# chenchen235/SemStereo

Measured on AMD Instinct MI355X. Metric: stereo pairs/sec, hot segment (gwc+concat volumes, 3-D hourglass stack, soft-argmax), 1024x1024 maxdisp=128, higher is better.
Workload: dtype f32; 1 GPU; BASELINE.json configs[1]: 1024x1024, maxdisp=128, batch=1/GPU x 1 GPU(s); features [B,128,H/4,W/4]+[B,256,H/8,W/8] -> disparity; input_sets_rotated=3, execution=steps round-robin on 6 HIP streams (PairPipeline); bit-identical to one stream, conv_engine=f16x3, hip_graph=False

## Files before the change

### include/semstereo_hip.h

```cpp
#ifndef SEMSTEREO_HIP_H
#define SEMSTEREO_HIP_H

#ifdef __cplusplus
extern "C" {
#endif

typedef void* ss_stream_t;

enum ss_status {
    SS_OK = 0,
    SS_ERR_INVALID = -1,
    SS_ERR_UNSUPPORTED = -2,
    SS_ERR_LAUNCH = -3
};

int ss_abi_version(void);
int ss_reload_tuning(void);
int ss_set_fill_hint(int pairs_in_flight);
int ss_get_fill_hint(void);
const char* ss_status_string(int status);
const char* ss_last_hip_error(void);


int ss_groupwise_correlation_fwd(const float* fea1, const float* fea2, float* out,
                                 int B, int C, int H, int W, int groups, int normalize,
                                 ss_stream_t stream);

int ss_gwc_volume_fwd(const float* ref, const float* tgt, float* out,
                      int B, int C, int H, int W, int dmin, int ndisp, int groups, int normalize,
                      ss_stream_t stream);
int ss_gwc_patch_gate_fwd(const float* ref, const float* tgt, const float* patch_w, const float* gate_logits, float* out,
                          int B, int C, int H, int W, int dmin, int ndisp, int groups, int normalize, ss_stream_t stream);
int ss_gwc_volume_bwd(const float* grad_out, const float* ref, const float* tgt,
                      float* grad_ref, float* grad_tgt,
                      int B, int C, int H, int W, int dmin, int ndisp, int groups,
                      ss_stream_t stream);

int ss_concat_volume_fwd(const float* ref, const float* tgt, float* out,
                         int B, int C, int H, int W, int dmin, int ndisp, int mask_left, ss_stream_t stream);
int ss_concat_volume_bwd(const float* grad_out, float* grad_ref, float* grad_tgt,
                         int B, int C, int H, int W, int dmin, int ndisp, int mask_left, ss_stream_t stream);

int ss_warp_sampled_fwd(const float* x, const float* y, const float* disp,
                        float* y_warped, float* x_warped,
                        int B, int C, int H, int W, int nd, ss_stream_t stream);
int ss_warp_sampled_bwd(const float* grad_y_warped, const float* grad_x_warped, const float* y, const float* disp,
                        float* grad_x, float* grad_y, float* grad_disp, int B, int C, int H, int W, int nd,
                        ss_stream_t stream);
int ss_concat_sampled_fwd(const float* left, const float* right, const float* disp, const float* att,
                          float* out, int B, int C, int H, int W, int nd, ss_stream_t stream);
int ss_concat_sampled_bwd(const float* grad_out, const float* left, const float* right, const float* disp, const float* att,
                          float* grad_left, float* grad_right, float* grad_att, int B, int C, int H, int W, int nd, int margin,
                          ss_stream_t stream);
int ss_concat_sampled_presplit_fwd(const float* right, const float* disp, const float* att, void* xs, int* xexp,
                                   int B, int C, int H, int W, int nd, ss_stream_t stream);
int ss_stem_left_fwd(const float* q, const float* att, float* out, int B, int Cout, int nd, int H, int W,
                     ss_stream_t stream);
int ss_stem_left_fused_fwd(const float* left, const void* wsplit, const float* att, float* out, int B, int C,
                           int Cout, int nd, int H, int W, int nterms, ss_stream_t stream);
int ss_warp_correlation_fwd(const float* x, const float* y, const float* disp, float* out,
                            int B, int C, int H, int W, int nd, ss_stream_t stream);

int ss_disparity_regression_fwd(const float* prob, float* out, int B, int dmin, int ndisp, int H, int W,
                                ss_stream_t stream);
int ss_disparity_regression_bwd(const float* grad_out, float* grad_prob, int B, int dmin, int ndisp, int H, int W,
                                ss_stream_t stream);
int ss_disparity_variance_fwd(const float* prob, const float* disparity, float* out,
                              int B, int dmin, int ndisp, int H, int W, ss_stream_t stream);
int ss_softmax_regression_fwd(const float* logits, float* prob, float* disp, float* var,
                              int B, int dmin, int ndisp, int H, int W, ss_stream_t stream);
int ss_upsample_softmax_regression_fwd(const float* coarse, float* up, float* disp, float* var,
                                       int B, int dmin, int ndisp, int H, int W, ss_stream_t stream);

int ss_sample_strength_fwd(const float* left, const float* right, const float* pred0, const float* var,
                           const float* gamma, const float* beta, float* strength,
                           int B, int C, int H, int W, ss_stream_t stream);
int ss_topk_candidates_fwd(const float* logits, const float* strength, float* samples, float* att_topk,
                           float* pred_att, int B, int dmin, int ndisp, int H, int W, int k, ss_stream_t stream);

int ss_regression_topk_fwd(const float* cost, const float* samples, float* out,
                           int B, int nd, int H, int W, int k, ss_stream_t stream);
int ss_regression_topk_bwd(const float* grad_out, const float* cost, const float* samples, float* grad_cost,
                           float* grad_samples, int B, int nd, int H, int W, int k, ss_stream_t stream);

int ss_ssr_upsample_fwd(const float* depth_low, const float* weights, const float* pred_label,
                        const float* params, float* out, int B, int h, int w, int num_classes,
                        ss_stream_t stream);
int ss_ssr_param_count(void);
int ss_ssr_upsample_train_fwd(const float* depth_low, const float* weights, const float* pred_label, const float* params,
                              float* out, float* saved, float* rm0, float* rv0, long long* nbt0, float* rma, float* rva,
                              long long* nbta, float* rm1, float* rv1, long long* nbt1, float* rm2, float* rv2, long long* nbt2,
                              float eps0, float epsa, float eps1, float eps2, double mom0, double moma, double mom1, double mom2,
                              int batch_stats, int B, int h, int w, int num_classes, double* workspace, long long workspace_bytes,
                              ss_stream_t stream);
int ss_ssr_upsample_train_bwd(const float* depth_low, const float* weights, const float* pred_label, const float* params,
                              const float* saved, const float* grad_out, float* grad_depth_low, float* grad_weights,
                              float* grad_pred_label, float* grad_params, int batch_stats, int B, int h, int w, int num_classes,
                              double* workspace, long long workspace_bytes, ss_stream_t stream);

int ss_channel_gate_fwd(const float* att_logits, const float* cv, float* out,
                        int B, int C, int D, int H, int W, ss_stream_t stream);

int ss_channel_att_logits_fwd(const float* im, const void* w1_split, const float* scale1, const float* shift1,
                              const void* w2_split, const float* bias2, float* out,
                              int B, int Cin, int Cmid, int Cout, int H, int W, int sigmoid, ss_stream_t stream);

int ss_conv3d_fwd(const float* in, const float* wpack, const float* scale, const float* shift,
                  const float* residual, const float* gate, float* out,
                  int B, int Cin, int D, int H, int W, int Cout, int k, int stride, int relu,
                  ss_stream_t stream);
int ss_conv3d_bf16s_fwd(const float* in, const void* wsplit, const float* scale, const float* shift,
                        const float* residual, const float* gate, float* out,
// ... 167 lines not shown
```

### semstereo_amd/_lib.py

```python
import ctypes
import os

import torch

_HERE = os.path.dirname(os.path.abspath(__file__))
LIB_PATH = os.path.join(_HERE, "csrc", "libsemstereo_hip.so")
ABI_VERSION = 20

_P = ctypes.c_void_p
_I = ctypes.c_int

_SIGNATURES = {
    "ss_groupwise_correlation_fwd": [_P, _P, _P, _I, _I, _I, _I, _I, _I, _P],
    "ss_gwc_volume_fwd": [_P, _P, _P, _I, _I, _I, _I, _I, _I, _I, _I, _P],
    "ss_gwc_patch_gate_fwd": [_P, _P, _P, _P, _P, _I, _I, _I, _I, _I, _I, _I, _I, _P],
    "ss_gwc_volume_bwd": [_P, _P, _P, _P, _P, _I, _I, _I, _I, _I, _I, _I, _P],
    "ss_concat_volume_fwd": [_P, _P, _P, _I, _I, _I, _I, _I, _I, _I, _P],
    "ss_concat_volume_bwd": [_P, _P, _P, _I, _I, _I, _I, _I, _I, _I, _P],
    "ss_warp_sampled_fwd": [_P, _P, _P, _P, _P, _I, _I, _I, _I, _I, _P],
    "ss_warp_sampled_bwd": [_P, _P, _P, _P, _P, _P, _P, _I, _I, _I, _I, _I, _P],
    "ss_concat_sampled_fwd": [_P, _P, _P, _P, _P, _I, _I, _I, _I, _I, _P],
    "ss_concat_sampled_bwd": [_P, _P, _P, _P, _P, _P, _P, _P, _I, _I, _I, _I, _I, _I, _P],
    "ss_concat_sampled_presplit_fwd": [_P, _P, _P, _P, _P, _I, _I, _I, _I, _I, _P],
    "ss_conv3d_presplit_fwd": [_P, _P, _P, _P, _P, _P, _P, _P, _I, _I, _I, _I, _I, _I, _I, _P],
    "ss_stem_left_fwd": [_P, _P, _P, _I, _I, _I, _I, _I, _P],
    "ss_stem_left_fused_fwd": [_P, _P, _P, _P, _I, _I, _I, _I, _I, _I, _I, _P],
    "ss_warp_correlation_fwd": [_P, _P, _P, _P, _I, _I, _I, _I, _I, _P],
    "ss_disparity_regression_fwd": [_P, _P, _I, _I, _I, _I, _I, _P],
    "ss_disparity_regression_bwd": [_P, _P, _I, _I, _I, _I, _I, _P],
    "ss_disparity_variance_fwd": [_P, _P, _P, _I, _I, _I, _I, _I, _P],
    "ss_softmax_regression_fwd": [_P, _P, _P, _P, _I, _I, _I, _I, _I, _P],
    "ss_upsample_softmax_regression_fwd": [_P, _P, _P, _P, _I, _I, _I, _I, _I, _P],
    "ss_regression_topk_fwd": [_P, _P, _P, _I, _I, _I, _I, _I, _P],
    "ss_regression_topk_bwd": [_P, _P, _P, _P, _P, _I, _I, _I, _I, _I, _P],
    "ss_sample_strength_fwd": [_P, _P, _P, _P, _P, _P, _P, _I, _I, _I, _I, _P],
    "ss_topk_candidates_fwd": [_P, _P, _P, _P, _P, _I, _I, _I, _I, _I, _I, _P],
    "ss_channel_gate_fwd": [_P, _P, _P, _I, _I, _I, _I, _I, _P],
    "ss_channel_att_logits_fwd": [_P, _P, _P, _P, _P, _P, _P, _I, _I, _I, _I, _I, _I, _I, _P],
    "ss_ssr_upsample_fwd": [_P, _P, _P, _P, _P, _I, _I, _I, _I, _P],
    "ss_ssr_upsample_train_fwd": [_P, _P, _P, _P, _P, _P] + [_P] * 12 + [ctypes.c_float] * 4 + [ctypes.c_double] * 4
                                 + [_I, _I, _I, _I, _I, _P, ctypes.c_longlong, _P],
    "ss_ssr_upsample_train_bwd": [_P] * 10 + [_I, _I, _I, _I, _I, _P, ctypes.c_longlong, _P],
    "ss_conv3d_fwd": [_P, _P, _P, _P, _P, _P, _P, _I, _I, _I, _I, _I, _I, _I, _I, _I, _P],
    "ss_conv3d_bf16s_fwd": [_P, _P, _P, _P, _P, _P, _P, _I, _I, _I, _I, _I, _I, _I, _I, _I, _P],
    "ss_conv3d_bf16s_partial_fwd": [_P, _P, _P, _P, _P, _P, _P, _I, _I, _I, _I, _I, _I, _I, _I, _P],
    "ss_conv3d_gather_fwd": [_P, _P, _P, _P, _P, _P, _P, _P, _P, _I, _I, _I, _I, _I, _I, _I, _I, _P],
    "ss_pack_conv3d_weights_bf16s": [_P, _P, _I, _I, _P],
    "ss_pack_conv3d_weights_f16s": [_P, _P, _I, _I, _P],
    "ss_conv2d_bf16s_fwd": [_P, _P, _P, _P, _P, _P, _I, _I, _I, _I, _I, _I, _I, _P],
    "ss_conv2d_bf16s_pair_fwd": [_P, _P, _P, _P, _P, _P, _I, _I, _I, _I, _I, _I, _I, _P],
    "ss_pack_conv2d_weights_bf16s": [_P, _P, _I, _I, _P],
    "ss_conv2d_bf16s_cat_fwd": [_P, _P, _P, _P, _P, _P, _P, _P, _I, _I, _I, _I, _I, _I, _I, _I, _P],
    "ss_deconv2d_bf16s_fwd": [_P, _P, _P, _P, _P, _I, _I, _I, _I, _I, _I, _I, _P],
    "ss_deconv2d_bf16s_pair_fwd": [_P, _P, _P, _P, _P, _P, _I, _I, _I, _I, _I, _I, _I, _P],
    "ss_pack_deconv2d_weights_f16s": [_P, _P, _I, _I, _P],
    "ss_pack_conv2d_weights_f16s": [_P, _P, _I, _I, _P],
    "ss_conv2d_k1_f16s_fwd": [_P, _P, _P, _P, _P, _I, _I, ctypes.c_longlong, _I, _I, _P],
    "ss_conv2d_k1_f16s_pair_fwd": [_P, _P, _P, _P, _P, _P, _I, _I, ctypes.c_longlong, _I, _I, _P],
    "ss_pack_conv2d_k1_weights_f16s": [_P, _P, _I, _I, _P],
    "ss_seghead_logits_fwd": [_P, _P, _P, _P, _P, _P, _P, _I, _I, _I, _I, _I, _P],
    "ss_pack_seghead_weights_f16s": [_P, _P, _I, _P],
    "ss_bilinear_up2_fwd": [_P, _P, _I, _I, _I, _I, _P],
    "ss_conv3d_head_bf16s_fwd": [_P, _P, _P, _P, _P, _I, _I, _I, _I, _I, _I, _I, _P],
    "ss_conv3d_head_bf16s_cl_fwd": [_P, _P, _P, _P, _P, _I, _I, _I, _I, _I, _I, _I, _P],
    "ss_conv3d_bf16s_cl_fwd": [_P, _P, _P, _P, _P, _I, _I, _I, _I, _I, _I, _I, _I, _P],
    "ss_pack_classifier_head_weights": [_P, _P, _P],
    "ss_conv3d_classifier_fused_fwd": [_P, _P, _P, _P, _P, _P, _P, _I, _I, _I, _I, _I, _I, _P],
    "ss_regression_topk_patched_fwd": [_P, _P, _P, _I, _I, _I, _I, _I, _P],
    "ss_pack_conv3d_head_weights_bf16s": [_P, _P, _I, _P],
    "ss_pack_conv3d_head_weights_f16s": [_P, _P, _I, _P],
    "ss_conv3d_pointwise_bf16s_fwd": [_P, _P, _P, _P, _P, _I, _I, _I, ctypes.c_longlong, _I, _I, _P],
    "ss_pack_pointwise_weights_bf16s": [_P, _P, _I, _I, _P],
    "ss_deconv3d_fwd": [_P, _P, _P, _P, _P, _P, _P, _P, _P, _I, _I, _I, _I, _I, _I, _I, _I, _P],
    "ss_pack_deconv3d_weights_f16s": [_P, _P, _I, _I, _P],
    "ss_deconv3d_bf16s_fwd": [_P, _P, _P, _P, _P, _P, _I, _I, _I, _I, _I, _I, _I, _I, _I, _P],
    "ss_pack_deconv3d_weights_bf16s": [_P, _P, _I, _I, _I, _P],
    "ss_pack_conv3d_weights": [_P, _P, _I, _I, _I, _I, _P],
    "ss_conv3d_wgrad_fwd": [_P, _P, _P, _I, _I, _I, _I, _I, _I, _I, _P],
    "ss_conv3d_wgrad_bf16s_fwd": [_P, _P, _P, _P, _I, _I, _I, _I, _I, _I, _I, _P],
# ... 107 lines not shown
```

### semstereo_amd/csrc/stem_left.hip

```cpp
#include <algorithm>

#include "common.h"
#include "split_bf16.h"

namespace {

constexpr int TH = 8, TW = 32, COG = 4;

template <int ND>
__global__ __launch_bounds__(256) void stem_left_kernel(const float* __restrict__ q, const float* __restrict__ att,
                                                         float* __restrict__ out, int Cout, int H, int W) {
    __shared__ float atile[ND][TH + 2][TW + 2];
    const int tid = threadIdx.x, tx = tid & 31, ty = tid >> 5;
    const int w0 = blockIdx.x * TW, h0 = blockIdx.y * TH;
    const int ngroups = Cout / COG;
    const int b = blockIdx.z / ngroups, co0 = (blockIdx.z % ngroups) * COG;
    const size_t plane = (size_t)H * W;
    const float* ab = att + (size_t)b * ND * plane;
    for (int e = tid; e < ND * (TH + 2) * (TW + 2); e += 256) {
        const int x = e % (TW + 2);
        int r = e / (TW + 2);
        const int y = r % (TH + 2), j = r / (TH + 2);
        const int gh = h0 + y - 1, gw = w0 + x - 1;
        atile[j][y][x] = ((unsigned)gh < (unsigned)H && (unsigned)gw < (unsigned)W) ? ab[(size_t)j * plane + (size_t)gh * W + gw] : 0.f;
    }
    __syncthreads();
    const int h = h0 + ty, w = w0 + tx;
    if (h >= H || w >= W) return;
    float acc[COG][ND];
#pragma unroll
    for (int c = 0; c < COG; ++c)
#pragma unroll
        for (int j = 0; j < ND; ++j) acc[c][j] = 0.f;
    const float* qb = q + ((size_t)b * 27 * Cout + co0) * plane;
    float qv[2][3][COG];
    auto load_q = [&](float (&dst)[3][COG], int s) {
        const int kh = s / 3, kw = s % 3;
        const int y = min(max(h + kh - 1, 0), H - 1), x = min(max(w + kw - 1, 0), W - 1);
        const float* p = qb + (size_t)y * W + x;
#pragma unroll
        for (int kd = 0; kd < 3; ++kd)
#pragma unroll
            for (int c = 0; c < COG; ++c) dst[kd][c] = p[((size_t)((kd * 3 + kh) * 3 + kw) * Cout + c) * plane];
    };
    load_q(qv[0], 0);
#pragma unroll
    for (int s = 0; s < 9; ++s) {
        if (s + 1 < 9) load_q(qv[(s + 1) & 1], s + 1);
        const int kh = s / 3, kw = s % 3;
        float a[ND + 2];
        a[0] = 0.f;
        a[ND + 1] = 0.f;
#pragma unroll
        for (int j = 0; j < ND; ++j) a[1 + j] = atile[j][ty + kh][tx + kw];
#pragma unroll
        for (int kd = 0; kd < 3; ++kd)
// ... 164 lines not shown
                const int qrow = ((kd * 3 + kh) * 3 + kw) * 2;
                const f32x2_t v = {qtile[qrow][hp], qtile[qrow + 1][hp]};
#pragma unroll
                for (int j = 0; j < NJ; ++j) o[j] = __builtin_elementwise_fma(f32x2_t{av[j + kd], av[j + kd]}, v, o[j]);
            }
        }
        if (inside) {
            float* ob = out + (((size_t)b * Cout + 2 * g) * ND + j0) * plane + (size_t)h * W + w;
#pragma unroll
            for (int j = 0; j < NJ; ++j) {
                ob[(size_t)j * plane] = o[j][0];
                ob[((size_t)ND + j) * plane] = o[j][1];
            }
        }
    }
}

template <int ND>
int launch_fused(const float* left, const void* wsplit, const float* att, float* out, int B, int Cout, int H, int W,
                 int nterms, hipStream_t st) {
    const size_t lds = ((size_t)(ND + 2) * HH * HW + 64 * QCOLS) * sizeof(float);
    dim3 grid(ss::ceil_div(W, FTW), ss::ceil_div(H, FTH), B);
    if (nterms == 6) {
        auto kern = stem_left_fused<ND, 6>;
        if (lds > 64 * 1024) {
            if (ss::ensure_dynamic_lds(reinterpret_cast<const void*>(kern), (int)lds) != SS_OK) return SS_ERR_LAUNCH;
        }
        hipLaunchKernelGGL(kern, grid, dim3(256), lds, st, left, reinterpret_cast<const uint4*>(wsplit), att, out, Cout, H, W);
    } else {
        auto kern = stem_left_fused<ND, 3>;
        if (lds > 64 * 1024) {
            if (ss::ensure_dynamic_lds(reinterpret_cast<const void*>(kern), (int)lds) != SS_OK) return SS_ERR_LAUNCH;
        }
        hipLaunchKernelGGL(kern, grid, dim3(256), lds, st, left, reinterpret_cast<const uint4*>(wsplit), att, out, Cout, H, W);
    }
    return ss::check_launch();
}

}

extern "C" int ss_stem_left_fused_fwd(const float* left, const void* wsplit, const float* att, float* out, int B, int C,
                                      int Cout, int nd, int H, int W, int nterms, ss_stream_t stream) {
    SS_REQUIRE(left && wsplit && att && out);
    SS_REQUIRE(B > 0 && C > 0 && Cout > 0 && nd > 0 && H > 0 && W > 0 && (nterms == 3 || nterms == 6));
    SS_REQUIRE((reinterpret_cast<uintptr_t>(wsplit) & 15) == 0);
    if (C != 32 || Cout % 2 != 0 || B > 65535) return SS_ERR_UNSUPPORTED;
    if ((long long)C * H * W * 4 >= 0x7fffffffLL || (long long)nd * H * W * 4 >= 0x7fffffffLL) return SS_ERR_UNSUPPORTED;
    hipStream_t st = ss::as_stream(stream);
    if (nd == 24) return launch_fused<24>(left, wsplit, att, out, B, Cout, H, W, nterms, st);
    if (nd == 32) return launch_fused<32>(left, wsplit, att, out, B, Cout, H, W, nterms, st);
    if (nd == 6) return launch_fused<6>(left, wsplit, att, out, B, Cout, H, W, nterms, st);
    return SS_ERR_UNSUPPORTED;
}
```

### semstereo_amd/engine.py

```python
import os
import weakref

import torch
import torch.nn as nn

from . import _lib, ops
from ._lib import call, ptr

PATH_COUNTS = {"hip": 0, "torch": 0}


def _inference(module, *tensors):
    if module.training:
        return False
    if torch.is_grad_enabled():
        if any(t is not None and t.requires_grad for t in tensors):
            return False
        if any(p.requires_grad for p in module.parameters()):
            return False
        if module.__dict__.get("_is_replica", False):
            for m in module.modules():
                if any(p is not None and p.requires_grad for p in getattr(m, "_former_parameters", {}).values()):
                    return False
    return True
# ... 562 lines not shown
    w = w.detach().float().reshape(w.shape[0], w.shape[1]).contiguous()
    _lib.require_device(w)
    Cout, Cin = w.shape
    assert Cin % 16 == 0
    out = torch.empty(((Cout + 31) // 32) * (Cin // 16) * 3 * 2 * 32 * 8, dtype=torch.int16, device=w.device)
    with torch.cuda.device(w.device):
        call("ss_pack_pointwise_weights_bf16s", ptr(w), ptr(out), Cout, Cin)
    return out


def conv3d_pointwise_bf16s_hip(x, wsplit, Cout, scale, shift, relu, nterms):
    x = x if x.is_contiguous() else x.contiguous()
    dev = _lib.require_device(x, scale, shift)
    B, Cin = x.shape[0], x.shape[1]
    out = torch.empty((B, Cout) + tuple(x.shape[2:]), dtype=x.dtype, device=x.device)
    with torch.cuda.device(dev):
        call("ss_conv3d_pointwise_bf16s_fwd", ptr(x), ptr(wsplit), ptr(scale), ptr(shift), ptr(out), B, Cin, Cout,
             x[0, 0].numel(), int(relu), int(nterms))
    return out


def _conv_geometry(conv):
    k, s, p = conv.kernel_size, conv.stride, conv.padding
    assert k[0] == k[1] == k[2] and s[0] == s[1] == s[2] and p[0] == p[1] == p[2] == k[0] // 2
    assert conv.bias is None and conv.groups == 1 and conv.dilation == (1, 1, 1)
    return k[0], s[0]


def run_convbn(owner, key, conv, bn, x, relu, residual=None, gate=None):
    k, s = _conv_geometry(conv)
    if CONV_ENGINE != "f32" and k == 3 and s in (1, 2) and conv.out_channels > 1:
        nterms = _tiled_nterms()
        ws, scale, shift = _packed_affine(owner, key + ("/f16s" if nterms == 19 else "/bf16s"), conv, bn,
                                          lambda w: pack_conv_weight_bf16s(w, nterms))
        return conv3d_bf16s_hip(x, ws, conv.out_channels, scale, shift, relu, nterms, residual, gate, stride=s)
    if (CONV_ENGINE != "f32" and k == 3 and s == 1 and conv.out_channels == 1 and conv.in_channels in (16, 32, 64)
            and residual is None and gate is None):
        nterms = _head_nterms()
        ws, scale, shift = _packed_affine(owner, key + "/head_%d" % nterms, conv, bn, lambda w: pack_head_weight_bf16s(w, nterms))
        return conv3d_head_bf16s_hip(x, ws, scale, shift, relu, nterms)
    wp, scale, shift = _packed_affine(owner, key, conv, bn, pack_conv_weight)
    return conv3d_hip(x, wp, scale, shift, k, s, relu, residual, gate)


TRAIN_HIP = os.environ.get("SS_TRAIN_HIP", "1") != "0"
SSR_TRAIN_HIP = os.environ.get("SS_SSR_TRAIN_HIP", "1") != "0"
LOSS_HIP = os.environ.get("SS_LOSS_HIP", "1") != "0"
METRICS_HIP = os.environ.get("SS_METRICS_HIP", "1") != "0"
CLASSIFIER_CL = os.environ.get("SS_CLASSIFIER_CL", "1") != "0"
CLASSIFIER_FUSED = os.environ.get("SS_CLASSIFIER_FUSED", "1") != "0"


STEM_LEFT_FUSED = os.environ.get("SS_STEM_LEFT_FUSED", "1") != "0"


def _stem_halves_params(stem, C):
    conv, bn = stem.conv, stem.bn if stem.use_bn else None
    Cout = conv.out_channels
    assert conv.in_channels == 2 * C and _conv_geometry(conv) == (3, 1)
    srcs = [conv.weight] + ([bn.weight, bn.bias, bn.running_mean, bn.running_var] if bn is not None else [])

    def build():
        sc, sh = fold_bn(bn) if bn is not None else (None, None)
        w = conv.weight.detach().float()
        wl = w[:, :C].reshape(Cout, C, 27)
        wq = wl.permute(2, 0, 1).reshape(27 * Cout, C)
        wf = torch.zeros(Cout // 2, 64, C, dtype=w.dtype, device=w.device)
        wf[:, :54] = wl.reshape(Cout // 2, 2, C, 27).permute(0, 3, 1, 2).reshape(Cout // 2, 54, C)
        return (pack_pointwise_weight_bf16s(wq), pack_pointwise_weight_bf16s(wf.reshape(Cout // 2 * 64, C)),
                pack_conv_weight_bf16s(w[:, C:].contiguous(), _tiled_nterms()), sc, sh)
    return _cache(stem).get("bc/halves/" + CONV_ENGINE, srcs, build)


def stem_broadcast_half(stem, left, att):
    assert stem.is_3d and not stem.deconv and CONV_ENGINE != "f32" and _inference(stem, left, att)
    C, Cout = left.shape[1], stem.conv.out_channels
    nterms = _aux_nterms()
    wq, wf, _, _, _ = _stem_halves_params(stem, C)
    PATH_COUNTS["hip"] += 1
    if C == 32 and Cout % 2 == 0 and STEM_LEFT_FUSED:
        return ops.stem_left_fused(left, wf, att, Cout, nterms)
    q = conv3d_pointwise_bf16s_hip(left, wq, 27 * Cout, None, None, False, nterms)
    return ops.stem_left(q, att)


def stem_volume_half(stem, right_vol, partial, gate=None):
    assert stem.is_3d and not stem.deconv and CONV_ENGINE != "f32" and _inference(stem, right_vol, partial, gate)
    nterms = _tiled_nterms()
    _, _, wr, scale, shift = _stem_halves_params(stem, right_vol.shape[1])
    g = None if gate is None else gate.contiguous()
    return conv3d_bf16s_hip(right_vol, wr, stem.conv.out_channels, scale, shift, bool(stem.relu), nterms, None, g, partial=partial)


STEM_PRESPLIT = os.environ.get("SS_STEM_PRESPLIT", "0") != "0"


def stem_presplit_applies(stem, right):
    return (STEM_PRESPLIT and CONV_ENGINE == "f16x3" and right.shape[1] % 8 == 0 and stem.conv.in_channels == 2 * right.shape[1]
            and _conv_geometry(stem.conv) == (3, 1))


def stem_volume_half_presplit(stem, xs, xexp, partial, gate=None):
    assert stem.is_3d and not stem.deconv and CONV_ENGINE == "f16x3" and _inference(stem, partial, gate)
    B, nchunks, _, D, H, W, _ = xs.shape
    _, _, wr, scale, shift = _stem_halves_params(stem, nchunks * 8)
    Cout = stem.conv.out_channels
    g = None if gate is None else gate.contiguous()
    dev = _lib.require_device(partial, scale, shift, g)
    out = torch.empty((B, Cout, D, H, W), dtype=torch.float32, device=xs.device)
    if partial is not None:
        assert partial.shape == out.shape and partial.is_contiguous()
    with torch.cuda.device(dev if dev is not None else xs.device):
        call("ss_conv3d_presplit_fwd", ptr(xs), ptr(xexp), ptr(wr), ptr(partial), ptr(scale), ptr(shift), ptr(g), ptr(out),
             B, nchunks * 8, D, H, W, Cout, int(bool(stem.relu)))
    return out


STEM_GATHER = os.environ.get("SS_STEM_GATHER", "1") != "0"
STEM_INPLACE = os.environ.get("SS_STEM_INPLACE", "1") != "0"


def stem_gather_applies(stem, right, samples):
    return (STEM_GATHER and CONV_ENGINE == "f16x3" and right.shape[1] % 8 == 0 and right.shape[1] >= 16
            and stem.conv.in_channels == 2 * right.shape[1] and _conv_geometry(stem.conv) == (3, 1)
            and right.dtype == torch.float32 and samples.dtype == torch.float32
            and right.shape[-1] > 1 and right.shape[-2] > 1)


def stem_gather_half(stem, right, samples, att, partial, gate=None, consume_partial=False):
    assert stem.is_3d and not stem.deconv and CONV_ENGINE == "f16x3" and _inference(stem, right, partial, gate)
    right, samples = right.contiguous(), samples.contiguous()
    att = att.reshape(att.shape[0], att.shape[-3], att.shape[-2], att.shape[-1]).contiguous()
    B, C, H, W = right.shape
    nd = samples.shape[1]
    assert samples.shape == (B, nd, H, W) and att.shape == samples.shape
    _, _, wr, scale, shift = _stem_halves_params(stem, C)
    Cout = stem.conv.out_channels
    g = None if gate is None else gate.contiguous()
    dev = _lib.require_device(right, samples, att, partial, scale, shift, g)
    inplace = consume_partial and STEM_INPLACE and partial is not None and partial.is_contiguous() and tuple(partial.shape) == (B, Cout, nd, H, W) and not partial.requires_grad
    out = partial if inplace else torch.empty((B, Cout, nd, H, W), dtype=torch.float32, device=right.device)
    if partial is not None:
        assert partial.shape == out.shape and partial.is_contiguous()
    if g is not None:
        assert g.shape == (B, Cout, H, W)
    PATH_COUNTS["hip"] += 1
    with torch.cuda.device(dev):
        call("ss_conv3d_gather_fwd", ptr(right), ptr(samples), ptr(att), ptr(wr), ptr(partial), ptr(scale), ptr(shift), ptr(g),
             ptr(out), B, C, nd, H, W, Cout, int(bool(stem.relu)), _tiled_nterms())
    return out


def stem_of_broadcast_and_volume(stem, left, att, right_vol, gate=None):
    return stem_volume_half(stem, right_vol, stem_broadcast_half(stem, left, att), gate)

ATTENTION_FORM = os.environ.get("SS_ATTENTION", "split")

SWITCHES = ("CONV_ENGINE", "DECONV_F16", "DECONV_MIN_WORKGROUPS", "DECONV_BF16S", "CLASSIFIER_CL", "CLASSIFIER_FUSED", "CLASSIFIER_FOLD", "TRAIN_HIP", "SSR_TRAIN_HIP", "LOSS_HIP", "METRICS_HIP", "ATTENTION_FORM",
            "STEM_LEFT_FUSED", "STEM_PRESPLIT", "STEM_GATHER", "STEM_INPLACE", "HEAD_F16", "CONV2D_HIP", "DECODER_HIP", "HEADS_HIP")
```

### semstereo_amd/ops.py

```python
import torch
import torch.nn.functional as F

from . import _lib
from . import deferred as dfr
from ._lib import call, ptr


def _c(t):
    return t if t.is_contiguous() else t.contiguous()


def _needs_grad(*ts):
    return torch.is_grad_enabled() and any(t is not None and t.requires_grad for t in ts)



def signed_range(maxdisp):
    return -int(maxdisp), 2 * int(maxdisp)


def unsigned_range(maxdisp):
    return 0, int(maxdisp)


# ... 377 lines not shown
def concat_volume_sampled(left, right, disparity_samples, att=None):
    right, disp = _c(right), _c(disparity_samples)
    left = None if left is None else _c(left)
    if att is not None:
        att = _c(att.reshape(att.shape[0], att.shape[-3], att.shape[-2], att.shape[-1]))
    dev = _lib.require_device(left, right, disp, att)
    B, C, H, W = right.shape
    nd = disp.shape[1]
    out = torch.empty((B, (2 if left is not None else 1) * C, nd, H, W), dtype=right.dtype, device=right.device)
    with torch.cuda.device(dev):
        call("ss_concat_sampled_fwd", ptr(left), ptr(right), ptr(disp), ptr(att), ptr(out), B, C, H, W, nd)
    return out


def concat_volume_sampled_presplit(right, disparity_samples, att=None):
    right, disp = _c(right), _c(disparity_samples)
    if att is not None:
        att = _c(att.reshape(att.shape[0], att.shape[-3], att.shape[-2], att.shape[-1]))
    dev = _lib.require_device(right, disp, att)
    B, C, H, W = right.shape
    nd = disp.shape[1]
    assert C % 8 == 0
    xs = torch.empty((B, C // 8, 2, nd, H, W, 8), dtype=torch.int16, device=right.device)
    xexp = torch.empty(3 * B, dtype=torch.int32, device=right.device)
    with torch.cuda.device(dev):
        call("ss_concat_sampled_presplit_fwd", ptr(right), ptr(disp), ptr(att), ptr(xs), ptr(xexp), B, C, H, W, nd)
    return xs, xexp


def stem_left(q, att):
    q = _c(q)
    att = _c(att.reshape(att.shape[0], att.shape[-3], att.shape[-2], att.shape[-1]))
    dev = _lib.require_device(q, att)
    B, nd, H, W = att.shape
    assert q.shape[0] == B and q.shape[1] % 27 == 0 and tuple(q.shape[2:]) == (H, W)
    Cout = q.shape[1] // 27
    out = torch.empty((B, Cout, nd, H, W), dtype=q.dtype, device=q.device)
    with torch.cuda.device(dev):
        call("ss_stem_left_fwd", ptr(q), ptr(att), ptr(out), B, Cout, nd, H, W)
    return out


def stem_left_fused(left, wsplit, att, Cout, nterms=6):
    left = _c(left)
    att = _c(att.reshape(att.shape[0], att.shape[-3], att.shape[-2], att.shape[-1]))
    dev = _lib.require_device(left, att)
    B, nd, H, W = att.shape
    out = torch.empty((B, Cout, nd, H, W), dtype=left.dtype, device=left.device)
    with torch.cuda.device(dev):
        call("ss_stem_left_fused_fwd", ptr(left), ptr(wsplit), ptr(att), ptr(out), B, left.shape[1], Cout, nd, H, W, int(nterms))
    return out


def warp_correlation(x, y, disparity_samples):
    x, y, disp = _c(x), _c(y), _c(disparity_samples)
    dev = _lib.require_device(x, y, disp)
    B, C, H, W = x.shape
    nd = disp.shape[1]
    out = torch.empty((B, nd, H, W), dtype=x.dtype, device=x.device)
    with torch.cuda.device(dev):
        call("ss_warp_correlation_fwd", ptr(x), ptr(y), ptr(disp), ptr(out), B, C, H, W, nd)
    return out


def sample_strength(left, right, pred0, var, gamma, beta):
    left, right, pred0, var = _c(left), _c(right), _c(pred0), _c(var)
    gamma, beta = _c(gamma.detach().reshape(1)), _c(beta.detach().reshape(1))
    dev = _lib.require_device(left, right, pred0, var, gamma, beta)
    B, C, H, W = left.shape
    assert pred0.shape == (B, H, W) and var.shape == (B, 1, H, W)
    out = torch.empty((B, 5, H, W), dtype=left.dtype, device=left.device)
    with torch.cuda.device(dev):
        call("ss_sample_strength_fwd", ptr(left), ptr(right), ptr(pred0), ptr(var), ptr(gamma), ptr(beta), ptr(out),
             B, C, H, W)
    return out


TOPK_CANDIDATES_MAX_D = 128


def topk_candidates(att_weights, strength, maxdisp, k, _range=None):
    att_weights, strength = _c(att_weights), _c(strength)
    dev = _lib.require_device(att_weights, strength)
    B, one, D, H, W = att_weights.shape
    dmin, nd = _range or signed_range(maxdisp)
    assert one == 1 and D == nd and strength.shape == (B, 5, H, W)
    samples = torch.empty((B, k, H, W), dtype=att_weights.dtype, device=att_weights.device)
    att_topk = torch.empty((B, 1, k, H, W), dtype=att_weights.dtype, device=att_weights.device)
    pred_att = torch.empty((B, H, W), dtype=att_weights.dtype, device=att_weights.device)
    with torch.cuda.device(dev):
        call("ss_topk_candidates_fwd", ptr(att_weights), ptr(strength), ptr(samples), ptr(att_topk), ptr(pred_att),
             B, dmin, nd, H, W, int(k))
    _mark_integer(samples, True)
    return att_topk, samples, pred_att


def _mark_integer(samples, verdict):
    samples._ss_integer = (bool(verdict), samples._version)


def integer_candidates(samples):
    mark = getattr(samples, "_ss_integer", None)
    if mark is not None and mark[1] == samples._version:
        return mark[0]
    if samples.is_cuda and torch.cuda.is_current_stream_capturing():
        return False
# ... 46 lines not shown
```

Before: 618.1 pairs/s.

## Add MFMA f16-split kernel for stem left-half broadcast convolution

Adds a new stem-left kernel for C=Cout=32 that runs the left-feature 3x3 spatial contraction on MFMA 32x32x16 f16 instructions. It uses a three-product hi/lo split with per-tile exponent scaling and per-row weight unscale factors, then folds the depth taps against the attention volume with packed FMAs. A packing kernel prepares weight fragments that are cached alongside the existing stem params. This replaces the scalar or bf16s fused path for nd in {6,24,32} when the f16x3 engine is active. The goal is to cut ALU cost of the stem's left half, at the price of extra precision handling and the complexity of a new kernel.

Result: faster. 628.2 pairs/s, median of 6 (+1.6%).

```diff
diff --git a/include/semstereo_hip.h b/include/semstereo_hip.h
--- a/include/semstereo_hip.h
+++ b/include/semstereo_hip.h
@@ -58,6 +58,9 @@
                      ss_stream_t stream);
 int ss_stem_left_fused_fwd(const float* left, const void* wsplit, const float* att, float* out, int B, int C,
                            int Cout, int nd, int H, int W, int nterms, ss_stream_t stream);
+int ss_stem_left_mfma_fwd(const float* left, const void* wsplit, const float* att, float* out, int B, int C,
+                          int Cout, int nd, int H, int W, ss_stream_t stream);
+int ss_pack_stem_left_weights_f16s(const float* w, void* wsplit, int Cout, int C, ss_stream_t stream);
 int ss_warp_correlation_fwd(const float* x, const float* y, const float* disp, float* out,
                             int B, int C, int H, int W, int nd, ss_stream_t stream);
 
diff --git a/semstereo_amd/_lib.py b/semstereo_amd/_lib.py
--- a/semstereo_amd/_lib.py
+++ b/semstereo_amd/_lib.py
@@ -25,6 +25,8 @@
     "ss_conv3d_presplit_fwd": [_P, _P, _P, _P, _P, _P, _P, _P, _I, _I, _I, _I, _I, _I, _I, _P],
     "ss_stem_left_fwd": [_P, _P, _P, _I, _I, _I, _I, _I, _P],
     "ss_stem_left_fused_fwd": [_P, _P, _P, _P, _I, _I, _I, _I, _I, _I, _I, _P],
+    "ss_stem_left_mfma_fwd": [_P, _P, _P, _P, _I, _I, _I, _I, _I, _I, _P],
+    "ss_pack_stem_left_weights_f16s": [_P, _P, _I, _I, _P],
     "ss_warp_correlation_fwd": [_P, _P, _P, _P, _I, _I, _I, _I, _I, _P],
     "ss_disparity_regression_fwd": [_P, _P, _I, _I, _I, _I, _I, _P],
     "ss_disparity_regression_bwd": [_P, _P, _I, _I, _I, _I, _I, _P],
diff --git a/semstereo_amd/csrc/stem_left.hip b/semstereo_amd/csrc/stem_left.hip
--- a/semstereo_amd/csrc/stem_left.hip
+++ b/semstereo_amd/csrc/stem_left.hip
@@ -2,6 +2,7 @@
 
 #include "common.h"
 #include "split_bf16.h"
+#include "split_f16.h"
 
 namespace {
 
@@ -272,3 +273,215 @@
     if (nd == 6) return launch_fused<6>(left, wsplit, att, out, B, Cout, H, W, nterms, st);
     return SS_ERR_UNSUPPORTED;
 }
+
+namespace {
+
+constexpr int MROWS = 8;
+constexpr int NCG = 32 / MROWS;
+constexpr int WFRAG_HALVES = NCG * 9 * 2 * 2 * 64 * 8;
+
+template <int ND>
+__global__ __launch_bounds__(256, 2) void stem_left_mfma(const float* __restrict__ left, const uint4* __restrict__ wfrag,
+                                                          const float4* __restrict__ winv, const float* __restrict__ att,
+                                                          float* __restrict__ out, int H, int W) {
+    constexpr int C = 32, Cout = 32;
+    __shared__ __attribute__((aligned(16))) float atile_s[ND + 2][HH][HW];
+    __shared__ uint4 ltile[8][NPOSH];
+    __shared__ float4 uinv[NCG * 9 * 2 * 3];
+    __shared__ unsigned wmax[4];
+    float (*atile)[HH][HW] = atile_s + 1;
+    const int tid = threadIdx.x, lane = tid & 63, wave = tid >> 6;
+    const int l31 = lane & 31, half = lane >> 5;
+    const int w0 = blockIdx.x * FTW, h0 = blockIdx.y * FTH, b = blockIdx.z;
+    const size_t plane = (size_t)H * W;
+
+    {
+        const __amdgpu_buffer_rsrc_t ares = __builtin_amdgcn_make_buffer_rsrc(
+            const_cast<float*>(att + (size_t)b * ND * plane), 0, (int)min((long long)ND * (long long)plane * 4, 0x7fffffffLL), 0x00020000);
+        constexpr int NE = (ND * NPOSH + 255) / 256;
+        float av[NE];
+#pragma unroll
+        for (int k = 0; k < NE; ++k) {
+            const int e = tid + 256 * k;
+            const int x = e % HW;
+            int r = e / HW;
+            const int y = r % HH, j = r / HH;
+            const int gh = h0 + y - 1, gw = w0 + x - 1;
+            const bool ok = e < ND * NPOSH && (unsigned)gh < (unsigned)H && (unsigned)gw < (unsigned)W;
+            av[k] = __builtin_bit_cast(float, __builtin_amdgcn_raw_buffer_load_b32(
+                                                  ares, (int)(ok ? (unsigned)(((size_t)j * plane + (size_t)gh * W + gw) * 4) : 0x80000000u), 0, 0));
+        }
+#pragma unroll
+        for (int k = 0; k < NE; ++k) {
+            const int e = tid + 256 * k;
+            if (e < ND * NPOSH) (&atile[0][0][0])[e] = av[k];
+        }
+        if (tid < NPOSH) {
+            (&atile[-1][0][0])[tid] = 0.f;
+            (&atile[ND][0][0])[tid] = 0.f;
+        }
+    }
+
+    if (tid < NCG * 9 * 2 * 3) uinv[tid] = winv[tid];
+
+    int e_tile;
+    {
+        const __amdgpu_buffer_rsrc_t lres = __builtin_amdgcn_make_buffer_rsrc(
+            const_cast<float*>(left + (size_t)b * C * plane), 0, (int)min((long long)C * (long long)plane * 4, 0x7fffffffLL), 0x00020000);
+        const int chan_b = (int)(plane * 4);
+        constexpr int NS = (4 * NPOSH + 255) / 256;
+        float x[NS][8];
+        float m = 0.f;
+#pragma unroll
+        for (int k = 0; k < NS; ++k) {
+            const int e = tid + 256 * k;
+            const int p = e % NPOSH, oct = e / NPOSH;
+            const int gh = h0 + p / HW - 1, gw = w0 + p % HW - 1;
+            const bool ok = e < 4 * NPOSH && (unsigned)gh < (unsigned)H && (unsigned)gw < (unsigned)W;
+            const unsigned off = ok ? (unsigned)((8LL * oct * plane + (size_t)gh * W + gw) * 4) : 0x80000000u;
+#pragma unroll
+            for (int j = 0; j < 8; ++j)
+                x[k][j] = __builtin_bit_cast(float, __builtin_amdgcn_raw_buffer_load_b32(lres, (int)off, j * chan_b, 0));
+            m = abs_max<false>(x[k], m);
+        }
+        const unsigned wm = wave_max_bits(__float_as_uint(m));
+        if (lane == 0) wmax[wave] = wm;
+        __syncthreads();
+        e_tile = workgroup_exponent(wmax);
+        const float sc = scale_for(e_tile);
+#pragma unroll
+        for (int k = 0; k < NS; ++k) {
+            const int e = tid + 256 * k;
+            if (e >= 4 * NPOSH) continue;
+            const int p = e % NPOSH, oct = e / NPOSH;
+            unsigned hi[4], lo[4];
+#pragma unroll
+            for (int j = 0; j < 4; ++j) split2_pk_f16(x[k][2 * j] * sc, x[k][2 * j + 1] * sc, hi[j], lo[j]);
+            ltile[oct * 2 + 0][p] = make_uint4(hi[0], hi[1], hi[2], hi[3]);
+            ltile[oct * 2 + 1][p] = make_uint4(lo[0], lo[1], lo[2], lo[3]);
+        }
+    }
+    __syncthreads();
+
+    const float unl = unscale_for(e_tile);
+    const int h = h0 + wave, w = w0 + l31;
+    const bool inside = h < H && w < W;
+    uint4 wa[4], wn[4];
+    auto load_w = [&](uint4 (&wd)[4], int step) {
+        const uint4* wf = wfrag + (size_t)step * 4 * 64 + lane;
+#pragma unroll
+        for (int k = 0; k < 4; ++k) wd[k] = wf[k * 64];
+    };
+    load_w(wa, 0);
+#pragma unroll 1
+    for (int cg = 0; cg < NCG; ++cg) {
+        f32x2_t o[2][ND];
+#pragma unroll
+        for (int pr = 0; pr < 2; ++pr)
+#pragma unroll
+            for (int j = 0; j < ND; ++j) o[pr][j] = f32x2_t{0.f, 0.f};
+#pragma unroll 1
+        for (int s = 0; s < 9; ++s) {
+            load_w(wn, min(cg * 9 + s + 1, NCG * 9 - 1));
+            const int kh = s / 3, kw = s - 3 * kh;
+            const int hp = (wave + kh) * HW + l31 + kw;
+            f32x16 acc;
+#pragma unroll
+            for (int r = 0; r < 16; ++r) acc[r] = 0.f;
+#pragma unroll
+            for (int ks = 0; ks < 2; ++ks) {
+                const f16x8 a0 = __builtin_bit_cast(f16x8, wa[ks * 2 + 0]);
+                const f16x8 a1 = __builtin_bit_cast(f16x8, wa[ks * 2 + 1]);
+                const f16x8 b0 = __builtin_bit_cast(f16x8, ltile[(ks * 2 + half) * 2 + 0][hp]);
+                const f16x8 b1 = __builtin_bit_cast(f16x8, ltile[(ks * 2 + half) * 2 + 1][hp]);
+                acc = __builtin_amdgcn_mfma_f32_32x32x16_f16(a1, b0, acc, 0, 0, 0);
+                acc = __builtin_amdgcn_mfma_f32_32x32x16_f16(a0, b1, acc, 0, 0, 0);
+                acc = __builtin_amdgcn_mfma_f32_32x32x16_f16(a0, b0, acc, 0, 0, 0);
+            }
+            const float* ap = &atile[0][0][0] + hp;
+            float av[ND + 2];
+#pragma unroll
+            for (int j = -1; j <= ND; ++j) av[1 + j] = ap[j * NPOSH];
+#pragma unroll
+            for (int kd = 0; kd < 3; ++kd) {
+                const float4 u = uinv[((cg * 9 + s) * 2 + half) * 3 + kd];
+                const f32x2_t v0 = {acc[kd * 4 + 0] * unl * u.x, acc[kd * 4 + 1] * unl * u.y};
+                const f32x2_t v1 = {acc[kd * 4 + 2] * unl * u.z, acc[kd * 4 + 3] * unl * u.w};
+#pragma unroll
+                for (int j = 0; j < ND; ++j) {
+                    const f32x2_t a = {av[j + kd], av[j + kd]};
+                    o[0][j] = __builtin_elementwise_fma(a, v0, o[0][j]);
+                    o[1][j] = __builtin_elementwise_fma(a, v1, o[1][j]);
+                }
+            }
+#pragma unroll
+            for (int k = 0; k < 4; ++k) wa[k] = wn[k];
+        }
+        if (inside) {
+            float* ob = out + (((size_t)b * Cout + cg * MROWS + half * 4) * ND) * plane + (size_t)h * W + w;
+#pragma unroll
+            for (int pr = 0; pr < 2; ++pr)
+#pragma unroll
+                for (int j = 0; j < ND; ++j) {
+                    ob[((size_t)(2 * pr) * ND + j) * plane] = o[pr][j][0];
+                    ob[((size_t)(2 * pr + 1) * ND + j) * plane] = o[pr][j][1];
+                }
+        }
+    }
+}
+
+__global__ __launch_bounds__(256) void pack_stem_left_f16s_kernel(const float* __restrict__ w, unsigned short* __restrict__ wsplit,
+                                                                   float* __restrict__ winv) {
+    const int t = blockIdx.x * 256 + threadIdx.x;
+    if (t >= NCG * 9 * 32) return;
+    const int row = t % 32, s = (t / 32) % 9, cg = t / (32 * 9);
+    const int kd = row / MROWS, c8 = row % MROWS;
+    const bool live = kd < 3;
+    const float* wr = w + ((size_t)(cg * MROWS + c8) * 32) * 27 + kd * 9 + s;
+    float m = 0.f;
+    if (live)
+        for (int c = 0; c < 32; ++c) m = fmaxf(m, fabsf(wr[c * 27]));
+    const float u = unscale_for(max((int)(__float_as_uint(m) >> 23), E_MIN));
+    if (live) winv[((cg * 9 + s) * 2 + c8 / 4) * 12 + kd * 4 + c8 % 4] = u;
+    for (int c = 0; c < 32; ++c) {
+        const int ks = c / 16, hf = (c / 8) % 2, j = c % 8;
+        const float x = live ? wr[c * 27] / u : 0.f;
+#pragma unroll
+        for (int term = 0; term < 2; ++term)
+            wsplit[((((size_t)(cg * 9 + s) * 2 + ks) * 2 + term) * 64 + hf * 32 + row) * 8 + j] = split_weight_f16(x, term);
+    }
+}
+
+template <int ND>
+int launch_mfma(const float* left, const void* wsplit, const float* att, float* out, int B, int H, int W, hipStream_t st) {
+    const float4* winv = reinterpret_cast<const float4*>(reinterpret_cast<const unsigned short*>(wsplit) + WFRAG_HALVES);
+    dim3 grid(ss::ceil_div(W, FTW), ss::ceil_div(H, FTH), B);
+    hipLaunchKernelGGL(stem_left_mfma<ND>, grid, dim3(256), 0, st, left, reinterpret_cast<const uint4*>(wsplit), winv, att, out, H, W);
+    return ss::check_launch();
+}
+
+}
+
+extern "C" int ss_stem_left_mfma_fwd(const float* left, const void* wsplit, const float* att, float* out, int B, int C,
+                                     int Cout, int nd, int H, int W, ss_stream_t stream) {
+    SS_REQUIRE(left && wsplit && att && out);
+    SS_REQUIRE(B > 0 && C > 0 && Cout > 0 && nd > 0 && H > 0 && W > 0);
+    SS_REQUIRE((reinterpret_cast<uintptr_t>(wsplit) & 15) == 0);
+    if (C != 32 || Cout != 32 || B > 65535 || ss::ceil_div(H, FTH) > 65535) return SS_ERR_UNSUPPORTED;
+    if ((long long)C * H * W * 4 >= 0x7fffffffLL || (long long)nd * H * W * 4 >= 0x7fffffffLL) return SS_ERR_UNSUPPORTED;
+    hipStream_t st = ss::as_stream(stream);
+    if (nd == 24) return launch_mfma<24>(left, wsplit, att, out, B, H, W, st);
+    if (nd == 32) return launch_mfma<32>(left, wsplit, att, out, B, H, W, st);
+    if (nd == 6) return launch_mfma<6>(left, wsplit, att, out, B, H, W, st);
+    return SS_ERR_UNSUPPORTED;
+}
+
+extern "C" int ss_pack_stem_left_weights_f16s(const float* w, void* wsplit, int Cout, int C, ss_stream_t stream) {
+    SS_REQUIRE(w && wsplit);
+    SS_REQUIRE((reinterpret_cast<uintptr_t>(wsplit) & 15) == 0);
+    if (C != 32 || Cout != 32) return SS_ERR_UNSUPPORTED;
+    unsigned short* ws = reinterpret_cast<unsigned short*>(wsplit);
+    hipLaunchKernelGGL(pack_stem_left_f16s_kernel, dim3(ss::ceil_div(NCG * 9 * 32, 256)), dim3(256), 0, ss::as_stream(stream), w, ws,
+                       reinterpret_cast<float*>(ws + WFRAG_HALVES));
+    return ss::check_launch();
+}
diff --git a/semstereo_amd/engine.py b/semstereo_amd/engine.py
--- a/semstereo_amd/engine.py
+++ b/semstereo_amd/engine.py
@@ -638,6 +638,11 @@
 
 
 STEM_LEFT_FUSED = os.environ.get("SS_STEM_LEFT_FUSED", "1") != "0"
+STEM_LEFT_MFMA = os.environ.get("SS_STEM_LEFT_MFMA", "1") != "0"
+
+
+def stem_left_takes_mfma(C, Cout, nd):
+    return CONV_ENGINE == "f16x3" and STEM_LEFT_FUSED and STEM_LEFT_MFMA and C == 32 and Cout == 32 and nd in (6, 24, 32)
 
 
 def _stem_halves_params(stem, C):
@@ -653,8 +658,9 @@
         wq = wl.permute(2, 0, 1).reshape(27 * Cout, C)
         wf = torch.zeros(Cout // 2, 64, C, dtype=w.dtype, device=w.device)
         wf[:, :54] = wl.reshape(Cout // 2, 2, C, 27).permute(0, 3, 1, 2).reshape(Cout // 2, 54, C)
+        wm = ops.pack_stem_left_weights_f16s(wl) if CONV_ENGINE == "f16x3" and C == 32 and Cout == 32 else None
         return (pack_pointwise_weight_bf16s(wq), pack_pointwise_weight_bf16s(wf.reshape(Cout // 2 * 64, C)),
-                pack_conv_weight_bf16s(w[:, C:].contiguous(), _tiled_nterms()), sc, sh)
+                pack_conv_weight_bf16s(w[:, C:].contiguous(), _tiled_nterms()), sc, sh, wm)
     return _cache(stem).get("bc/halves/" + CONV_ENGINE, srcs, build)
 
 
@@ -662,8 +668,10 @@
     assert stem.is_3d and not stem.deconv and CONV_ENGINE != "f32" and _inference(stem, left, att)
     C, Cout = left.shape[1], stem.conv.out_channels
     nterms = _aux_nterms()
-    wq, wf, _, _, _ = _stem_halves_params(stem, C)
+    wq, wf, _, _, _, wm = _stem_halves_params(stem, C)
     PATH_COUNTS["hip"] += 1
+    if stem_left_takes_mfma(C, Cout, att.shape[-3]):
+        return ops.stem_left_mfma(left, wm, att, Cout)
     if C == 32 and Cout % 2 == 0 and STEM_LEFT_FUSED:
         return ops.stem_left_fused(left, wf, att, Cout, nterms)
     q = conv3d_pointwise_bf16s_hip(left, wq, 27 * Cout, None, None, False, nterms)
@@ -673,7 +681,7 @@
 def stem_volume_half(stem, right_vol, partial, gate=None):
     assert stem.is_3d and not stem.deconv and CONV_ENGINE != "f32" and _inference(stem, right_vol, partial, gate)
     nterms = _tiled_nterms()
-    _, _, wr, scale, shift = _stem_halves_params(stem, right_vol.shape[1])
+    _, _, wr, scale, shift, _ = _stem_halves_params(stem, right_vol.shape[1])
     g = None if gate is None else gate.contiguous()
     return conv3d_bf16s_hip(right_vol, wr, stem.conv.out_channels, scale, shift, bool(stem.relu), nterms, None, g, partial=partial)
 
@@ -689,7 +697,7 @@
 def stem_volume_half_presplit(stem, xs, xexp, partial, gate=None):
     assert stem.is_3d and not stem.deconv and CONV_ENGINE == "f16x3" and _inference(stem, partial, gate)
     B, nchunks, _, D, H, W, _ = xs.shape
-    _, _, wr, scale, shift = _stem_halves_params(stem, nchunks * 8)
+    _, _, wr, scale, shift, _ = _stem_halves_params(stem, nchunks * 8)
     Cout = stem.conv.out_channels
     g = None if gate is None else gate.contiguous()
     dev = _lib.require_device(partial, scale, shift, g)
@@ -720,7 +728,7 @@
     B, C, H, W = right.shape
     nd = samples.shape[1]
     assert samples.shape == (B, nd, H, W) and att.shape == samples.shape
-    _, _, wr, scale, shift = _stem_halves_params(stem, C)
+    _, _, wr, scale, shift, _ = _stem_halves_params(stem, C)
     Cout = stem.conv.out_channels
     g = None if gate is None else gate.contiguous()
     dev = _lib.require_device(right, samples, att, partial, scale, shift, g)
@@ -743,4 +751,4 @@
 ATTENTION_FORM = os.environ.get("SS_ATTENTION", "split")
 
 SWITCHES = ("CONV_ENGINE", "DECONV_F16", "DECONV_MIN_WORKGROUPS", "DECONV_BF16S", "CLASSIFIER_CL", "CLASSIFIER_FUSED", "CLASSIFIER_FOLD", "TRAIN_HIP", "SSR_TRAIN_HIP", "LOSS_HIP", "METRICS_HIP", "ATTENTION_FORM",
-            "STEM_LEFT_FUSED", "STEM_PRESPLIT", "STEM_GATHER", "STEM_INPLACE", "HEAD_F16", "CONV2D_HIP", "DECODER_HIP", "HEADS_HIP")
+            "STEM_LEFT_FUSED", "STEM_LEFT_MFMA", "STEM_PRESPLIT", "STEM_GATHER", "STEM_INPLACE", "HEAD_F16", "CONV2D_HIP", "DECODER_HIP", "HEADS_HIP")
diff --git a/semstereo_amd/ops.py b/semstereo_amd/ops.py
--- a/semstereo_amd/ops.py
+++ b/semstereo_amd/ops.py
@@ -453,6 +453,30 @@
     return out
 
 
+STEM_LEFT_MFMA_PACKED = 4 * 9 * 2 * 2 * 64 * 8 + 2 * 4 * 9 * 24
+
+
+def pack_stem_left_weights_f16s(wl):
+    wl = _c(wl.detach().float())
+    dev = _lib.require_device(wl)
+    assert tuple(wl.shape) == (32, 32, 27)
+    out = torch.empty(STEM_LEFT_MFMA_PACKED, dtype=torch.int16, device=wl.device)
+    with torch.cuda.device(dev):
+        call("ss_pack_stem_left_weights_f16s", ptr(wl), ptr(out), 32, 32)
+    return out
+
+
+def stem_left_mfma(left, wsplit, att, Cout):
+    left = _c(left)
+    att = _c(att.reshape(att.shape[0], att.shape[-3], att.shape[-2], att.shape[-1]))
+    dev = _lib.require_device(left, att)
+    B, nd, H, W = att.shape
+    out = torch.empty((B, Cout, nd, H, W), dtype=left.dtype, device=left.device)
+    with torch.cuda.device(dev):
+        call("ss_stem_left_mfma_fwd", ptr(left), ptr(wsplit), ptr(att), ptr(out), B, left.shape[1], Cout, nd, H, W)
+    return out
+
+
 def warp_correlation(x, y, disparity_samples):
     x, y, disp = _c(x), _c(y), _c(disparity_samples)
     dev = _lib.require_device(x, y, disp)
```
